# kkoutini/PaSST

Measured on AMD Instinct MI355X. Metric: clips/s (10s@32k) fwd+bwd passt_s, higher is better.
Workload: dtype bf16; 1 GPU; passt_s_swa_p16_128_ap476 train step (mel front end + mixup + fwd + BCE + bwd + adamw), 768/12/12, 474 tokens (s_patchout_t=40,f=4), random-init weights; global_batch=64, per_gpu_batch=64, parallelism=dp1, gemm_launch=persistent, 256 workgroups, input=waveform (B,1,320000) f32 resident in HBM

## Files before the change

### passt_amd/csrc/gemm.hip

```cpp
#include <algorithm>
#include <cstring>
#include <type_traits>

#include "pa_mma.h"

namespace pa {

static constexpr int NT_GROUP_M = 4;
static constexpr int BM = 128, BN = 128, KB = 128;
static constexpr int TILE_BYTES = BM * KB;
static constexpr int GEMM_LDS = 2 * 2 * TILE_BYTES;

#ifdef PA_PROBE
__device__ unsigned long long* g_probe_buf = nullptr;
static constexpr int PROBE_SLOTS = 512;
#define PA_PROBE_STAMP(cond, idx)                                                                             \
    do {                                                                                                      \
        if ((cond) && (wave & 3) == 0 && lane == 0 && (idx) < PROBE_SLOTS)                                    \
            ((unsigned long long*)(smem + G::LDS))[(wave >> 2) * PROBE_SLOTS + (idx)] = __builtin_amdgcn_s_memtime(); \
    } while (0)
#define PA_PROBE_FLAG(a, bit) (((a).reserved >> (bit)) & 1)
#define PA_PROBE_STAMP_TN(cond, idx)                                                                          \
    do {                                                                                                      \
        if ((cond) && (wave & 3) == 0 && lane == 0 && (idx) < PROBE_SLOTS)                                    \
// ... 588 lines not shown
        const int col = (c >> 1) * 32 + (c & 1) * 16 + 8 * h;
        const bool ok = col < ncols && !PA_PROBE_FLAG(a, 0);
        vo[c] = ok ? (uint32_t)q * ld2 + (uint32_t)col * 2u : V2_OOB;
        vo2[c] = ok ? (uint32_t)q * ld2b + (uint32_t)col * 2u : V2_OOB;
    }
    f32x4 b4[2][4];
#pragma unroll
    for (int j = 0; j < 2; ++j)
#pragma unroll
        for (int g = 0; g < 4; ++g) {
            b4[j][g] = f32x4{0.f, 0.f, 0.f, 0.f};
            if constexpr (EPI != PA_EPI_DGELU) {
                if (bias_row) b4[j][g] = *(const f32x4*)(bias_row + wc * 64 + j * 32 + 8 * g + 4 * h);
            }
        }
    float cs = 1.f;
    if constexpr (EPI == PA_EPI_STORE) {
        if (nb < a.colscale_n) {
            cs = a.colscale;
#pragma unroll
            for (int j = 0; j < 2; ++j)
#pragma unroll
                for (int g = 0; g < 4; ++g) b4[j][g] *= cs;
        }
    }
    constexpr int XD = V3Aux<EPI, TM>::PASSES > 0 ? V3Aux<EPI, TM>::PASSES : 1;
#pragma unroll
    for (int i = 0; i < TM; ++i) {
        __builtin_amdgcn_sched_barrier(0);
        uint32_t xg[2][4][2];
        if constexpr (EPI == PA_EPI_DGELU) {
#pragma unroll
            for (int c = 0; c < 4; ++c) {
                const u32x4 x = aux.v[(i % XD) * 4 + c];
                const int j = c >> 1, gp = c & 1;
                xg[j][2 * gp][0] = swap32_lo(x[0], x[2], xg[j][2 * gp + 1][0]);
                xg[j][2 * gp][1] = swap32_lo(x[1], x[3], xg[j][2 * gp + 1][1]);
            }
            __builtin_amdgcn_sched_barrier(0);
            if (i + XD < TM) aux.load_pass(i % XD, i + XD);
        }
#pragma unroll
        for (int j = 0; j < 2; ++j) {
            uint32_t w[4][2], w2[4][2];
#pragma unroll
            for (int g = 0; g < 4; ++g)
#pragma unroll
                for (int e2 = 0; e2 < 2; ++e2) {
                    const int r = 4 * g + 2 * e2;
                    f32x2 v = {acc[i][j][r] + b4[j][g][2 * e2], acc[i][j][r + 1] + b4[j][g][2 * e2 + 1]};
                    if constexpr (EPI == PA_EPI_STORE) v = f32x2{fmaf(acc[i][j][r], cs, b4[j][g][2 * e2]), fmaf(acc[i][j][r + 1], cs, b4[j][g][2 * e2 + 1])};
                    if constexpr (EPI == PA_EPI_DGELU) {
                        const uint32_t xw = xg[j][g][e2];
                        const f32x2 x = {__builtin_bit_cast(float, xw << 16), __builtin_bit_cast(float, xw & 0xffff0000u)};
                        v = v * (PA_PROBE_FLAG(a, 2) ? x : gelu_grad_fast2(x));
                    }
                    w[g][e2] = cvt_pk_bf16(v[0], v[1]);
                    if constexpr (EPI == PA_EPI_GELU) {
                        const f32x2 gl = PA_PROBE_FLAG(a, 2) ? v : gelu_fast2(v);
                        w2[g][e2] = cvt_pk_bf16(gl[0], gl[1]);
                    }
                }
#pragma unroll
            for (int gp = 0; gp < 2; ++gp) {
                uint32_t o0, o1;
                const uint32_t k0 = swap32_lo(w[2 * gp][0], w[2 * gp + 1][0], o0), k1 = swap32_lo(w[2 * gp][1], w[2 * gp + 1][1], o1);
                __builtin_amdgcn_raw_buffer_store_b128(u32x4{k0, k1, o0, o1}, ors, vo[2 * j + gp] + (uint32_t)(i * 32) * ld2, 0, 0);
                if constexpr (EPI == PA_EPI_GELU) {
                    const uint32_t g0 = swap32_lo(w2[2 * gp][0], w2[2 * gp + 1][0], o0), g1 = swap32_lo(w2[2 * gp][1], w2[2 * gp + 1][1], o1);
                    __builtin_amdgcn_raw_buffer_store_b128(u32x4{g0, g1, o0, o1}, ors2, vo2[2 * j + gp] + (uint32_t)(i * 32) * ld2b, 0, 0);
                }
            }
        }
    }
}

template <int TM, bool RS = false>
__device__ __forceinline__ void gemm_epilogue_v3_resid(const pa_gemm_args& a, f32x16 (&acc)[TM][2], const float* bias_row,
                                                       int m0, int n0, int wr, int wc, int lane, V3Aux<PA_EPI_RESID, TM, RS>& aux) {
    const int h = lane >> 5, q = lane & 31;
    const int mb = m0 + wr * (TM * 32), nb = n0 + wc * 64;
    if (mb >= a.M || nb >= a.N) return;
    const int ncols = a.N - nb;
    const uint32_t ldo4 = (uint32_t)a.ldo32 * 4u;
    const auto ors = tile_rsrc((const char*)a.out_f32 + ((int64_t)mb * a.ldo32 + nb) * 4, ((int64_t)(a.M - mb - 1) * a.ldo32 + ncols) * 4);
    uint32_t vo[4];
#pragma unroll
    for (int g = 0; g < 4; ++g) vo[g] = (uint32_t)q * ldo4 + (uint32_t)(8 * g + 4 * h) * 4u;
    constexpr int NH = 2 * TM, DEPTH = V3Aux<PA_EPI_RESID, TM, RS>::HALVES;
#pragma unroll
    for (int hp = 0; hp < NH; ++hp) {
        const int i = hp >> 1, j = hp & 1;
        __builtin_amdgcn_sched_barrier(0);
        f32x4 o[4];
        float f = 1.f;
        if constexpr (RS) f = __shfl(aux.rsv[i >> 1], (i & 1) * 32 + q, 64);
#pragma unroll
        for (int g = 0; g < 4; ++g) {
            const f32x4 b = bias_row ? *(const f32x4*)(bias_row + wc * 64 + j * 32 + 8 * g + 4 * h) : f32x4{0.f, 0.f, 0.f, 0.f};
            const f32x4 r = __builtin_bit_cast(f32x4, aux.v[(hp % DEPTH) * 4 + g]);
            const f32x4 ab = f32x4{acc[i][j][4 * g] + b[0], acc[i][j][4 * g + 1] + b[1], acc[i][j][4 * g + 2] + b[2], acc[i][j][4 * g + 3] + b[3]};
            if constexpr (RS) o[g] = __builtin_elementwise_fma(f32x4{f, f, f, f}, ab, r);
            else o[g] = ab + r;
        }
        __builtin_amdgcn_sched_barrier(0);
        if (hp + DEPTH < NH) aux.load_half(hp % DEPTH, hp + DEPTH, ncols);
#pragma unroll
        for (int g = 0; g < 4; ++g) {
            const uint32_t off = (j * 32 + 8 * g + 4 * h < ncols && !PA_PROBE_FLAG(a, 0)) ? vo[g] + (uint32_t)(i * 32) * ldo4 + (uint32_t)j * 128u : V2_OOB;
            __builtin_amdgcn_raw_buffer_store_b128(__builtin_bit_cast(u32x4, o[g]), ors, off, 0, 0);
        }
    }
}

template <int N> __device__ __forceinline__ void wait_vmcnt() { asm volatile("s_waitcnt vmcnt(%0)" ::"n"(N) : "memory"); }
template <int PER> __device__ __forceinline__ void wait_vm_groups(int k) {
    switch (k) {
        case 0: wait_vmcnt<0>(); break;
        case 1: wait_vmcnt<PER>(); break;
        case 2: wait_vmcnt<2 * PER>(); break;
        default: wait_vmcnt<3 * PER>(); break;
    }
}

__device__ __forceinline__ void tile_coords(int pid, int tiles_m, int tiles_n, int group_m, int& tm, int& tn) {
    const int per_group = group_m * tiles_n;
    const int g = pid / per_group;
    const int first = g * group_m;
    const int gm = min(tiles_m - first, group_m);
    const int r = pid - g * per_group;
    tm = first + r % gm;
    tn = r / gm;
}

template <int KBT> __device__ __forceinline__ int swz_rows(int row) {
    if constexpr (KBT == 128) return swz_f128(row);
    else return (row >> 2) & 3;
}

struct pa_gemm_args_rs : pa_gemm_args {
    const float* rowscale;
};
template <bool RS> using gemm_kargs = std::conditional_t<RS, pa_gemm_args_rs, pa_gemm_args>;
static constexpr int EPI_RESID_ROWSCALE = 5;
__host__ __device__ constexpr bool epi_rs(int epix) { return epix == EPI_RESID_ROWSCALE; }
__host__ __device__ constexpr int epi_base(int epix) { return epix == EPI_RESID_ROWSCALE ? (int)PA_EPI_RESID : epix; }
template <bool RS> __device__ __forceinline__ const float* rowscale_of(const gemm_kargs<RS>& a) {
    if constexpr (RS) return a.rowscale;
    else return nullptr;
}

template <typename T, int EPIX, int WM, int WN, int TM, int STAGES, int KBT = KB, int EPV = 0>
__global__ __launch_bounds__(WM * WN * 64) __attribute__((amdgpu_waves_per_eu((KBT == 64 || EPV) ? 2 : 1))) void gemm_nt_kernel(const gemm_kargs<epi_rs(EPIX)> a, const int tiles_m, const int tiles_n,
                                                               const int nwg, const int ksteps_per_split) {
    constexpr bool RS = epi_rs(EPIX);
    constexpr int EPI = epi_base(EPIX);
    static_assert(!RS || EPV == 0, "row factors: the first-generation epilogue");
    constexpr int TBM = WM * TM * 32, TBN = WN * 64;
    constexpr int A_BYTES = TBM * KBT, B_BYTES = TBN * KBT, STAGE_BYTES = A_BYTES + B_BYTES;
    constexpr int CPR = KBT / 16, NSUB = KBT / 32;
    constexpr int NW = WM * WN;
    constexpr int A_PER = (A_BYTES / 1024) / NW;
    constexpr int B_PER = (B_BYTES / 1024) / NW;
    constexpr int PER = A_PER + B_PER;
    static_assert(A_PER * NW * 1024 == A_BYTES && B_PER * NW * 1024 == B_BYTES, "tile must split evenly over the waves");
    extern __shared__ __attribute__((aligned(16))) char smem[];
    const int tid = threadIdx.x;
    const int lane = tid & 63;
    const int wave = __builtin_amdgcn_readfirstlane(tid >> 6);
    const int wr = wave / WN, wc = wave % WN;

    int tm, tn;
    tile_coords(xcd_swizzle(blockIdx.x, nwg), tiles_m, tiles_n, 1024 / TBM, tm, tn);
    const int m0 = tm * TBM, n0 = tn * TBN;
    const int ksteps_total = (int)((int64_t)a.K * sizeof(T) / KBT);
    const int ks_begin = blockIdx.y * ksteps_per_split;
    const int ks_end = min(ksteps_total, ks_begin + ksteps_per_split);
    const int nsteps = ks_end - ks_begin;

    const char* srcA[A_PER];
    const char* srcB[B_PER];
#pragma unroll
    for (int i = 0; i < A_PER; ++i) {
        const int q = (wave * A_PER + i) * 64 + lane;
        const int row = q / CPR;
        const int c = (q % CPR) ^ swz_rows<KBT>(row);
        const int gm = min(m0 + row, a.M - 1);
        srcA[i] = (const char*)a.A + ((int64_t)gm * a.lda) * sizeof(T) + c * 16 + (int64_t)ks_begin * KBT;
    }
#pragma unroll
    for (int i = 0; i < B_PER; ++i) {
        const int q = (wave * B_PER + i) * 64 + lane;
        const int row = q / CPR;
        const int c = (q % CPR) ^ swz_rows<KBT>(row);
        const int gn = min(n0 + row, a.N - 1);
        srcB[i] = (const char*)a.B + ((int64_t)gn * a.ldb) * sizeof(T) + c * 16 + (int64_t)ks_begin * KBT;
    }
    auto stage = [&](int buf, int step) {
        char* sA = smem + buf * STAGE_BYTES + wave * (A_PER * 1024);
        char* sB = smem + buf * STAGE_BYTES + A_BYTES + wave * (B_PER * 1024);
#pragma unroll
        for (int i = 0; i < A_PER; ++i)
            __builtin_amdgcn_global_load_lds(
                (const __attribute__((address_space(1))) void*)(srcA[i] + (int64_t)step * KBT),
                (__attribute__((address_space(3))) void*)(sA + i * 1024), 16, 0, 0);
#pragma unroll
        for (int i = 0; i < B_PER; ++i)
            __builtin_amdgcn_global_load_lds(
                (const __attribute__((address_space(1))) void*)(srcB[i] + (int64_t)step * KBT),
                (__attribute__((address_space(3))) void*)(sB + i * 1024), 16, 0, 0);
    };

    f32x16 acc[TM][2];
#pragma unroll
    for (int i = 0; i < TM; ++i)
#pragma unroll
        for (int j = 0; j < 2; ++j)
#pragma unroll
            for (int r = 0; r < 16; ++r) acc[i][j][r] = 0.f;

    const int rsw = swz_rows<KBT>(lane & 31);
    const int offA = (wr * (TM * 32) + (lane & 31)) * KBT;
    const int offB = (wc * 64 + (lane & 31)) * KBT;
    const int half = lane >> 5;

#pragma unroll
    for (int p = 0; p < STAGES - 1; ++p)
        if (p < nsteps) stage(p, p);
    float bias8[8];
    load_bias8<EPI>(a, n0, wc, lane, bias8);
    int buf = 0;
    for (int t = 0; t < nsteps; ++t) {
        wait_vm_groups<PER>(min(STAGES - 2, nsteps - 1 - t));
        __builtin_amdgcn_s_barrier();
        if (t + STAGES - 1 < nsteps) {
            int nb = buf + STAGES - 1;
            if (nb >= STAGES) nb -= STAGES;
            stage(nb, t + STAGES - 1);
        }
        const char* sA = smem + buf * STAGE_BYTES;
        const char* sB = sA + A_BYTES;
        typename Frag<T>::type fa[2][TM], fb[2][2];
        auto read_frags = [&](int slot, int ks) {
            const int coff = ((ks * 2 + half) ^ rsw) << 4;
#pragma unroll
            for (int i = 0; i < TM; ++i) fa[slot][i] = *(const typename Frag<T>::type*)(sA + offA + i * 32 * KBT + coff);
#pragma unroll
            for (int j = 0; j < 2; ++j) fb[slot][j] = *(const typename Frag<T>::type*)(sB + offB + j * 32 * KBT + coff);
        };
        read_frags(0, 0);
#pragma unroll
        for (int ks = 0; ks < NSUB; ++ks) {
            if (ks + 1 < NSUB) read_frags((ks + 1) & 1, ks + 1);
#pragma unroll
            for (int i = 0; i < TM; ++i)
#pragma unroll
                for (int j = 0; j < 2; ++j) mma32<T>(acc[i][j], fa[ks & 1][i], fb[ks & 1][j]);
        }
        if (++buf == STAGES) buf = 0;
    }
    if constexpr (EPV != 0) {
        constexpr bool BLK = EPV == 2;
        static_assert(sizeof(T) == 2 && EPI != PA_EPI_PARTIAL, "epilogue v2: bf16 operands, fused epilogues");
        static_assert(!BLK || EPI == PA_EPI_GELU || EPI == PA_EPI_DGELU, "blocked pre-activation: GELU / GELU' only");
        constexpr bool BLKX = BLK && (EPI == PA_EPI_GELU || EPI == PA_EPI_DGELU);
        V2Aux<EPI, TM, BLKX> aux;
        aux.issue(a, m0, n0, wr, wc, lane);
        __syncthreads();
        const float* brow = (EPI != PA_EPI_DGELU && a.bias) ? a.bias + n0 : nullptr;
        if constexpr (EPI == PA_EPI_RESID) gemm_epilogue_v2_resid<TM>(a, acc, smem + wave * 8192, brow, m0, n0, wr, wc, lane, aux);
        else gemm_epilogue_v2_bf16<EPI, TM, BLKX>(a, acc, smem + wave * 8192, brow, m0, n0, wr, wc, lane, tm * WM + wr, aux);
    } else {
        __syncthreads();
        gemm_epilogue<T, EPI, TM, RS>(a, acc, (float*)(smem + wave * SLAB_BYTES), m0, n0, blockIdx.y, wr, wc, lane, bias8, tm * WM + wr, rowscale_of<RS>(a));
    }
}

template <typename T, int EPI, int WM, int WN, int TM, int STAGES, int KBT = KB, int EPV = 0, bool RS = false>
static int launch_gemm_v(const gemm_kargs<RS>& a, hipStream_t st) {
    constexpr int TBM = WM * TM * 32, TBN = WN * 64;
    constexpr int LDS = STAGES * (TBM + TBN) * KBT;
    static_assert(LDS <= 160 * 1024, "LDS ring too large");
    static_assert(LDS >= WM * WN * 32 * 68 * 4, "epilogue slabs must fit");
    if constexpr (EPV != 0) {
        const int64_t lim = (int64_t)1 << 31;
        if ((int64_t)a.M * a.ldolp * 2 >= lim || (int64_t)a.M * a.ldolp2 * 2 >= lim || (int64_t)a.M * a.ldaux * 2 >= lim ||
            (int64_t)a.M * a.ldr * 4 >= lim || (int64_t)a.M * a.ldo32 * 4 >= lim || a.N % 64 || (EPI == PA_EPI_RESID && a.row_mod > 0))
            return EPV == 2 ? PA_EUNSUPPORTED : launch_gemm_v<T, EPI, WM, WN, TM, STAGES, KBT, 0>(a, st);
    }
    const int tiles_m = (int)cdiv(a.M, TBM), tiles_n = (int)cdiv(a.N, TBN);
    const int nwg = tiles_m * tiles_n;
    const int ksteps = (int)((int64_t)a.K * sizeof(T) / KBT);
    const int splits = EPI == PA_EPI_PARTIAL ? a.split_k : 1;
    const int per = (int)cdiv(ksteps, splits);
    static signed char lds_attr[64] = {0};
    static_assert(!RS || EPI == PA_EPI_RESID, "row factors: the residual epilogue only");
    constexpr int EPIX = RS ? EPI_RESID_ROWSCALE : EPI;
    (void)lds_attr_on_this_device((const void*)gemm_nt_kernel<T, EPIX, WM, WN, TM, STAGES, KBT, EPV>, LDS, lds_attr);
    hipLaunchKernelGGL((gemm_nt_kernel<T, EPIX, WM, WN, TM, STAGES, KBT, EPV>), dim3(nwg, splits), dim3(WM * WN * 64), LDS, st, a,
                       tiles_m, tiles_n, nwg, per);
    const int rc = check_launch();
    if (rc == PA_OK && EPI == PA_EPI_DGELU && a.colsum_out) return finish_gemm_colsum(a, tiles_m * WM, st);
    return rc;
}

template <int TM, bool A3> struct StaggerGeom {
    static constexpr int TBM = 64 * TM, TBN = 256;
    static constexpr int A_BYTES = TBM * KB, B_BYTES = TBN * KB, STAGE_BYTES = A_BYTES + B_BYTES;
    static constexpr int NA = A3 ? 3 : 2;
    static constexpr int RING = NA * A_BYTES + 2 * B_BYTES;
    __host__ __device__ static constexpr int a_off(int s) { return A3 ? s * A_BYTES : s * STAGE_BYTES; }
    __host__ __device__ static constexpr int b_off(int s) { return A3 ? 3 * A_BYTES + s * B_BYTES : s * STAGE_BYTES + A_BYTES; }
    static constexpr int SLAB = A3 ? 8192 : SLAB_BYTES;
    static constexpr int SLABS_IN_STAGE = STAGE_BYTES / SLAB_BYTES;
    static constexpr int SLABS_A = A_BYTES / 8192, SLABS_B = B_BYTES / 8192;
    static constexpr int EXTRA = A3 ? 8 - SLABS_A - SLABS_B : 8 - SLABS_IN_STAGE;
    static constexpr int BIAS_OFF = RING + EXTRA * SLAB;
    static constexpr int TAB_OFF = BIAS_OFF + 1024;
    static constexpr int MAX_ROUNDS = A3 ? 128 : 512;
    static constexpr int LDS = TAB_OFF + MAX_ROUNDS * 16;
};

template <typename T, int EPIX, int TM, bool A3 = false, bool BLK = false, bool TR = false>
__global__ __launch_bounds__(512) void gemm_nt_stagger_kernel(const gemm_kargs<epi_rs(EPIX)> a, const int tiles_m, const int tiles_n,
                                                              const int nwg, const int ksteps_per_split, const int total) {
    constexpr bool RS = epi_rs(EPIX);
    constexpr int EPI = epi_base(EPIX);
    using G = StaggerGeom<TM, A3>;
    static_assert(!RS || (sizeof(T) == 2 && EPI == PA_EPI_RESID && !BLK), "row factors: the bf16 residual epilogues (v2 / v3)");
    static_assert(!TR || (sizeof(T) == 2 && EPI != PA_EPI_PARTIAL && !BLK), "v3: bf16 operands, fused epilogues, row-major pre-activation");
    constexpr int WN = 4;
    constexpr int TBM = G::TBM, TBN = G::TBN;
    constexpr int A_PER = TM;
    constexpr int NA = G::NA, PDA = NA - 1;
    constexpr bool USE_V2 = sizeof(T) == 2 && EPI != PA_EPI_PARTIAL;
    static_assert(!A3 || (TM <= 3 && (USE_V2 || EPI == PA_EPI_PARTIAL)), "A3: LDS budget / 8 KiB slabs");
    extern __shared__ __attribute__((aligned(16))) char smem[];
    const int tid = threadIdx.x;
    const int lane = tid & 63;
    const int wave = __builtin_amdgcn_readfirstlane(tid >> 6);
    const int wr = wave / WN, wc = wave % WN;
    const int ksteps_total = (int)((int64_t)a.K * sizeof(T) / KB);
    const int nres = gridDim.x, bid = blockIdx.x;

    const int full_rounds = total / nres;
    const int my_rounds = full_rounds + (bid < total - full_rounds * nres ? 1 : 0);
    int4* tab = (int4*)(smem + G::TAB_OFF);
    for (int r = tid; r < my_rounds; r += 512) {
        const int n = min(total - r * nres, nres);
        const int item = r * nres + xcd_swizzle(bid, n);
        int tm, tn;
        const int sp = item / nwg;
        tile_coords(item - sp * nwg, tiles_m, tiles_n, NT_GROUP_M, tm, tn);
        tab[r] = make_int4(tm * TBM, tn * TBN, sp, 0);
    }
#ifdef PA_PROBE
    for (int i = tid; i < 2 * PROBE_SLOTS; i += 512) ((unsigned long long*)(smem + G::LDS))[i] = 0ull;
#endif
    __syncthreads();
    const char* baseA;
    const char* baseB;
    uint32_t voffA[A_PER], voffB[4];
    auto item_of = [&](int r, int& m0, int& n0, int& split) {
        const int4 e = tab[r];
        m0 = __builtin_amdgcn_readfirstlane(e.x);
        n0 = __builtin_amdgcn_readfirstlane(e.y);
        split = __builtin_amdgcn_readfirstlane(e.z);
        const int ks_begin = split * ksteps_per_split;
        return min(ksteps_total, ks_begin + ksteps_per_split) - ks_begin;
    };
    auto point_A = [&](int r) {
        int m0, n0, split;
        item_of(r, m0, n0, split);
        baseA = (const char*)a.A + (int64_t)m0 * a.lda * sizeof(T) + (int64_t)split * ksteps_per_split * KB;
#pragma unroll
        for (int i = 0; i < A_PER; ++i) {
            const int q = (wave * A_PER + i) * 64 + lane;
            const int row = q >> 3;
            const int c = (q & 7) ^ swz_f128(row);
            voffA[i] = (uint32_t)min(row, a.M - 1 - m0) * (uint32_t)(a.lda * (int)sizeof(T)) + c * 16;
        }
    };
    auto point_B = [&](int r) {
        int m0, n0, split;
        item_of(r, m0, n0, split);
        baseB = (const char*)a.B + (int64_t)n0 * a.ldb * sizeof(T) + (int64_t)split * ksteps_per_split * KB;
#pragma unroll
        for (int i = 0; i < 4; ++i) {
            const int q = (wave * 4 + i) * 64 + lane;
            const int row = q >> 3;
            const int c = (q & 7) ^ swz_f128(row);
            voffB[i] = (uint32_t)min(row, a.N - 1 - n0) * (uint32_t)(a.ldb * (int)sizeof(T)) + c * 16;
        }
    };
    auto dmaA = [&](int slot, int step) {
        char* sA = smem + G::a_off(slot) + wave * (A_PER * 1024);
        const char* sb = baseA + (int64_t)step * KB;
        (void)a;
#pragma unroll
        for (int i = 0; i < A_PER; ++i)
            __builtin_amdgcn_global_load_lds((const __attribute__((address_space(1))) void*)(sb + voffA[i]),
                                             (__attribute__((address_space(3))) void*)(sA + i * 1024), 16, 0, EPI == PA_EPI_RESID ? CP_DMA_A_RESID : 0);
    };
    auto dmaB = [&](int slot, int step) {
        char* sB = smem + G::b_off(slot) + wave * 4096;
        const char* sb = baseB + (int64_t)step * KB;
#pragma unroll
        for (int i = 0; i < 4; ++i)
            __builtin_amdgcn_global_load_lds((const __attribute__((address_space(1))) void*)(sb + voffB[i]),
                                             (__attribute__((address_space(3))) void*)(sB + i * 1024), 16, 0, 0);
    };

    const int rsw = swz_f128(lane);
    const int offA = (wr * (TM * 32) + (lane & 31)) * 128;
    const int offB = (wc * 64 + (lane & 31)) * 128;
    const int half = lane >> 5;

    int round = 0;
    int m0, n0, split;
    int nsteps = item_of(0, m0, n0, split);
    point_A(0);
    point_B(0);
    dmaA(0, 0);
    if constexpr (A3) dmaA(1, 1);
    dmaB(0, 0);
    asm volatile("s_waitcnt vmcnt(0)" ::: "memory");
    __builtin_amdgcn_s_barrier();
    int ia = 0, ib = 0;

    for (;;) {
        const bool have_next = round + 1 < my_rounds;
        constexpr bool HAS_BIAS = EPI != PA_EPI_PARTIAL && EPI != PA_EPI_DGELU;
        if constexpr (HAS_BIAS) {
            if (a.bias && wr == 0)
                __builtin_amdgcn_global_load_lds((const __attribute__((address_space(1))) void*)(a.bias + min(n0 + wc * 64 + lane, a.N - 1)),
                                                 (__attribute__((address_space(3))) void*)(smem + G::BIAS_OFF + wc * 256), 4, 0, 0);
        }
        f32x16 acc[TM][2];
        constexpr int AUX_EPI = USE_V2 ? EPI : PA_EPI_STORE;
        std::conditional_t<TR, V3Aux<AUX_EPI, TM, RS>, V2Aux<AUX_EPI, TM, BLK, RS>> aux;
        constexpr int AUXN = decltype(aux)::N;
        static_assert(V3Aux<AUX_EPI, TM, RS>::N == V2Aux<AUX_EPI, TM, false, RS>::N, "both epilogues leave the same number of loads in flight");
        const int cur_m0 = m0, cur_n0 = n0, cur_split = split;
        if (wr == 1) __builtin_amdgcn_s_barrier();
        PA_PROBE_STAMP(round < 24, round * 16);

        for (int t = 0; t < nsteps; ++t) {
            const char* sA = smem + G::a_off(ia);
            const char* sB = smem + G::b_off(ib);
            const bool last = t + 1 == nsteps;
            const bool fetchB = !last || have_next;
            if (last && have_next) point_B(round + 1);
            const int stepB = last ? 0 : t + 1;
            const int ta = t + PDA;
            const bool fetchA = ta < nsteps || have_next;
            if (ta == nsteps && have_next) point_A(round + 1);
            const int stepA = ta < nsteps ? ta : ta - nsteps;
            int slotA = ia + PDA;
            if (slotA >= NA) slotA -= NA;
            const int tail = (A3 && fetchA ? A_PER : 0) + (USE_V2 && AUXN > 0 && last ? AUXN : 0);
            auto wait_tile = [&]() {
                if (tail == 0) asm volatile("s_waitcnt vmcnt(0)" ::: "memory");
                else if (tail == A_PER) wait_vmcnt<A_PER>();
                else if (tail == AUXN) wait_vmcnt<(AUXN > 0 ? AUXN : 1)>();
                else wait_vmcnt<A_PER + AUXN>();
            };
            constexpr int NPH = 4;
#pragma unroll
            for (int ph = 0; ph < NPH; ++ph) {
                typename Frag<T>::type fa[TM], fb[2];
                const int coff = ((ph * 2 + half) ^ rsw) << 4;
#pragma unroll
                for (int i = 0; i < TM; ++i) fa[i] = *(const typename Frag<T>::type*)(sA + offA + i * 32 * 128 + coff);
#pragma unroll
                for (int j = 0; j < 2; ++j) fb[j] = *(const typename Frag<T>::type*)(sB + offB + j * 32 * 128 + coff);
                if constexpr (A3) {
                    if (ph == 0 && fetchB) dmaB(ib ^ 1, stepB);
                    if (ph == 1 && fetchA) dmaA(slotA, stepA);
                } else {
                    if (ph == 0 && fetchA) dmaA(slotA, stepA);
                    if (ph == 1 && fetchB) dmaB(ib ^ 1, stepB);
                }
                if constexpr (USE_V2 && AUXN > 0) {
                    if (last && ph == NPH / 2) aux.issue(a, cur_m0, cur_n0, wr, wc, lane, rowscale_of<RS>(a));
                }
                if (ph == NPH - 1 && wr == 1) wait_tile();
                asm volatile("s_waitcnt lgkmcnt(0)" ::: "memory");
                __builtin_amdgcn_sched_barrier(0);
                __builtin_amdgcn_s_barrier();
                __builtin_amdgcn_s_setprio(1);
                if (ph == 0 && t == 0) {
#pragma unroll
                    for (int i = 0; i < TM; ++i)
#pragma unroll
                        for (int j = 0; j < 2; ++j) mma32_first<T>(acc[i][j], TR ? fb[j] : fa[i], TR ? fa[i] : fb[j]);
                } else {
#pragma unroll
                    for (int i = 0; i < TM; ++i)
#pragma unroll
                        for (int j = 0; j < 2; ++j) mma32<T>(acc[i][j], TR ? fb[j] : fa[i], TR ? fa[i] : fb[j]);
                }
                __builtin_amdgcn_s_setprio(0);
                if (ph == NPH - 1 && wr == 0) wait_tile();
                __builtin_amdgcn_sched_barrier(0);
                __builtin_amdgcn_s_barrier();
            }
            if (++ia == NA) ia = 0;
            ib ^= 1;
            PA_PROBE_STAMP(round < 24 && t < 13, round * 16 + 1 + t);
        }
        if (wr == 0) __builtin_amdgcn_s_barrier();
        const int freeA = ia == 0 ? NA - 1 : ia - 1, freeB = ib ^ 1;
        char* slab_c;
        if constexpr (A3) {
            slab_c = wave < G::SLABS_A ? smem + G::a_off(freeA) + wave * 8192
                     : wave < G::SLABS_A + G::SLABS_B ? smem + G::b_off(freeB) + (wave - G::SLABS_A) * 8192
                                                      : smem + G::RING + (wave - G::SLABS_A - G::SLABS_B) * 8192;
        } else {
            slab_c = wave < G::SLABS_IN_STAGE ? smem + G::a_off(freeA) + wave * SLAB_BYTES
                                              : smem + G::RING + (wave - G::SLABS_IN_STAGE) * SLAB_BYTES;
        }
        float* slab = (float*)slab_c;
        if (PA_PROBE_FLAG(a, 1)) {
#pragma unroll
            for (int i = 0; i < TM; ++i)
#pragma unroll
                for (int j = 0; j < 2; ++j)
#pragma unroll
                    for (int r = 0; r < 16; ++r) asm volatile("" ::"v"(acc[i][j][r]));
        } else if constexpr (USE_V2) {
            const float* brow = HAS_BIAS && a.bias ? (const float*)(smem + G::BIAS_OFF) : nullptr;
            if constexpr (TR) {
                (void)slab;
                if constexpr (EPI == PA_EPI_RESID) gemm_epilogue_v3_resid<TM, RS>(a, acc, brow, cur_m0, cur_n0, wr, wc, lane, aux);
                else gemm_epilogue_v3_bf16<EPI, TM>(a, acc, brow, cur_m0, cur_n0, wr, wc, lane, aux);
            } else if constexpr (EPI == PA_EPI_RESID) gemm_epilogue_v2_resid<TM, RS>(a, acc, (char*)slab, brow, cur_m0, cur_n0, wr, wc, lane, aux);
            else gemm_epilogue_v2_bf16<EPI, TM, BLK>(a, acc, (char*)slab, brow, cur_m0, cur_n0, wr, wc, lane, (cur_m0 / TBM) * 2 + wr, aux);
        } else if constexpr (EPI == PA_EPI_RESID || EPI == PA_EPI_PARTIAL) {
            (void)slab;
            gemm_epilogue_f32_direct<EPI, TM>(a, acc, HAS_BIAS && a.bias ? (const float*)(smem + G::BIAS_OFF) : nullptr, cur_m0,
                                              cur_n0, cur_split, wr, wc, lane);
        } else {
            float bias8[8];
#pragma unroll
            for (int e = 0; e < 8; ++e) bias8[e] = 0.f;
            if constexpr (HAS_BIAS) {
                if (a.bias) {
                    const float* brow = (const float*)(smem + G::BIAS_OFF) + wc * 64 + (lane & 7) * 8;
                    const f32x4 lo = *(const f32x4*)brow, hi = *(const f32x4*)(brow + 4);
#pragma unroll
                    for (int e = 0; e < 4; ++e) { bias8[e] = lo[e]; bias8[4 + e] = hi[e]; }
                }
            }
            gemm_epilogue<T, EPI, TM>(a, acc, slab, cur_m0, cur_n0, cur_split, wr, wc, lane, bias8, (cur_m0 / TBM) * 2 + wr);
        }
        PA_PROBE_STAMP(round < 24, round * 16 + 15);
#ifdef PA_PROBE
        if (!have_next && g_probe_buf && blockIdx.x < 8) {
            __syncthreads();
            for (int i = tid; i < 2 * PROBE_SLOTS; i += 512)
                g_probe_buf[blockIdx.x * 2 * PROBE_SLOTS + i] = ((const unsigned long long*)(smem + G::LDS))[i];
        }
#endif
        if (!have_next) break;
        ++round;
        nsteps = item_of(round, m0, n0, split);
        point_A(round);
        point_B(round);
        asm volatile("s_waitcnt lgkmcnt(0)" ::: "memory");
        __builtin_amdgcn_s_barrier();
    }
}

static bool epilogue_v3_enabled() {
    static const bool on = [] { const char* e = getenv("PA_EPILOGUE_V3"); return e && atoi(e) != 0; }();
    return on;
}

template <typename T, int EPI, int TM, bool A3 = false, bool BLK = false, bool TR = false, bool RS = false>
static int launch_gemm_stagger(const gemm_kargs<RS>& a, hipStream_t st) {
    using G = StaggerGeom<TM, A3>;
    if constexpr (!TR && !BLK && sizeof(T) == 2 && EPI != PA_EPI_PARTIAL && !(EPI == PA_EPI_RESID && TM == 4)) {
        if ((epilogue_v3_enabled() || (a.reserved & PA_GEMM_EPILOGUE_V3)) && !(EPI == PA_EPI_DGELU && a.colsum_out) &&
            !(EPI == PA_EPI_RESID && a.row_mod > 0))
            return launch_gemm_stagger<T, EPI, TM, A3, false, true, RS>(a, st);
    }
    static_assert(G::LDS <= 160 * 1024, "LDS budget");
    const int tiles_m = (int)cdiv(a.M, 64 * TM), tiles_n = (int)cdiv(a.N, 256);
    const int nwg = tiles_m * tiles_n;
    const int ksteps = (int)((int64_t)a.K * sizeof(T) / KB);
    const int splits = EPI == PA_EPI_PARTIAL ? a.split_k : 1;
    const int per = (int)cdiv(ksteps, splits);
    const int total = nwg * splits;
    const int64_t lim = (int64_t)1 << 31;
    const bool big = (int64_t)a.M * a.ldolp * 2 >= lim || (int64_t)a.M * a.ldolp2 * 2 >= lim || (int64_t)a.M * a.ldaux * 2 >= lim ||
                     (int64_t)a.M * a.ldr * 4 >= lim || (int64_t)a.M * a.ldo32 * 4 >= lim;
    if (ksteps < 1 || (int64_t)(splits - 1) * per >= ksteps ||
        (sizeof(T) == 2 && EPI != PA_EPI_PARTIAL && (big || (EPI == PA_EPI_RESID && a.row_mod > 0))))
        return BLK ? PA_EUNSUPPORTED : launch_gemm_v<T, EPI, 2, 2, 2, 2, KB, 0, RS>(a, st);
    if constexpr (A3) {
        if (ksteps - (splits - 1) * per < 2 || per < 2 || cdiv(total, 256) > G::MAX_ROUNDS) return launch_gemm_stagger<T, EPI, TM, false, BLK, TR, RS>(a, st);
    } else {
        if (cdiv(total, 256) > G::MAX_ROUNDS) return BLK ? PA_EUNSUPPORTED : launch_gemm_v<T, EPI, 2, 2, 2, 2, KB, 0, RS>(a, st);
    }
#ifdef PA_PROBE
    constexpr int LDS_BYTES = G::LDS + 2 * PROBE_SLOTS * 8;
#else
    constexpr int LDS_BYTES = G::LDS;
#endif
    static_assert(LDS_BYTES <= 160 * 1024, "LDS budget (probe build)");
    static signed char lds_attr[64] = {0};
    static_assert(!RS || EPI == PA_EPI_RESID, "row factors: the residual epilogue only");
    constexpr int EPIX = RS ? EPI_RESID_ROWSCALE : EPI;
    (void)lds_attr_on_this_device((const void*)gemm_nt_stagger_kernel<T, EPIX, TM, A3, BLK, TR>, LDS_BYTES, lds_attr);
    static const bool persist_env = [] { const char* e = getenv("PA_NT_PERSISTENT"); return !e || atoi(e) != 0; }();
    const bool persistent = persist_env && !(a.reserved & PA_GEMM_NO_PERSIST);
    hipLaunchKernelGGL((gemm_nt_stagger_kernel<T, EPIX, TM, A3, BLK, TR>), dim3(persistent ? std::min(total, 256) : total), dim3(512), LDS_BYTES, st, a,
                       tiles_m, tiles_n, nwg, per, total);
    const int rc = check_launch();
    if (rc == PA_OK && EPI == PA_EPI_DGELU && a.colsum_out) return finish_gemm_colsum(a, tiles_m * 2, st);
    return rc;
}

static int pick_nt_variant(int M, int N, int K) {
    struct Cand { int id, bm, bn, slots; float rate_short, rate_long; };
    static const Cand r06[] = {
        {1, 128, 128, 512, 700.f, 870.f},
        {8, 128, 256, 256, 800.f, 950.f},
        {7, 192, 256, 256, 950.f, 1075.f},
        {6, 256, 256, 256, 930.f, 900.f},
    };
    static const Cand r01[] = {
        {1, 128, 128, 512, 750.f, 930.f},
        {8, 128, 256, 256, 650.f, 1000.f},
        {7, 192, 256, 256, 780.f, 1250.f},
        {6, 256, 256, 256, 800.f, 1150.f},
    };
    static const bool isolated_table = [] { const char* e = getenv("PA_NT_RATES"); return e && !strcmp(e, "r06"); }();
    const Cand (&cands)[4] = isolated_table ? r06 : r01;
    int best = 1;
    double best_cost = 1e30;
    for (const Cand& c : cands) {
        const int64_t tiles = cdiv(M, c.bm) * cdiv(N, c.bn);
        const double rounds = (double)cdiv(tiles, c.slots);
        const double rate = (K <= 1024 ? c.rate_short : c.rate_long) / c.slots;
        const double cost = rounds * (double)c.bm * c.bn / rate;
        if (cost < best_cost) { best_cost = cost; best = c.id; }
    }
    return best;
}

template <typename T, int EPI>
static int launch_gemm(const pa_gemm_args& a, hipStream_t st) {
    if constexpr (sizeof(T) == 4) return launch_gemm_v<T, EPI, 2, 2, 2, 2>(a, st);
    else {
        int v = a.tune ? a.tune : pick_nt_variant(a.M, a.N, a.K);
        static const bool a3 = [] { const char* e = getenv("PA_NT_A3"); return !e || atoi(e) != 0; }();
        if (!a.tune && a3 && EPI != PA_EPI_PARTIAL && (v == 7 || v == 8)) v += 10;
        if constexpr (EPI == PA_EPI_GELU || EPI == PA_EPI_DGELU) {
            if (a.reserved & PA_GEMM_BLOCKED_PRE) {
                if (a.N % 64 || blocked_pre_rows(a.M) * a.N * 2 >= ((int64_t)1 << 31)) return PA_EUNSUPPORTED;
                static const bool mlp_2wg = [] { const char* e = getenv("PA_NT_MLP_2WG"); return e && atoi(e) != 0; }();
                if (!a.tune && mlp_2wg && a.M >= 16384 && a.N >= 1024 && a.K <= (EPI == PA_EPI_DGELU ? 1024 : 768)) v = 3;
                switch (v) {
                    case 6: return launch_gemm_stagger<T, EPI, 4, false, true>(a, st);
                    case 7: return launch_gemm_stagger<T, EPI, 3, false, true>(a, st);
                    case 8: return launch_gemm_stagger<T, EPI, 2, false, true>(a, st);
                    case 17: return launch_gemm_stagger<T, EPI, 3, true, true>(a, st);
                    case 18: return launch_gemm_stagger<T, EPI, 2, true, true>(a, st);
                    case 3: return launch_gemm_v<T, EPI, 2, 2, 3, 2, KB, 2>(a, st);
                    case 9: return launch_gemm_v<T, EPI, 1, 4, 4, 3, 64, 2>(a, st);
                }
                return PA_EUNSUPPORTED;
            }
        }
        switch (v) {
            case 1: return launch_gemm_v<T, EPI, 2, 2, 2, 2>(a, st);
            case 2: return launch_gemm_v<T, EPI, 2, 4, 4, 2>(a, st);
            case 3: return launch_gemm_v<T, EPI, 2, 2, 3, 2>(a, st);
            case 9: return launch_gemm_v<T, EPI, 1, 4, 4, 3, 64>(a, st);
            case 13: if constexpr (EPI != PA_EPI_PARTIAL) return launch_gemm_v<T, EPI, 2, 2, 3, 2, KB, 1>(a, st); else return PA_EINVAL;
            case 19: if constexpr (EPI != PA_EPI_PARTIAL) return launch_gemm_v<T, EPI, 1, 4, 4, 3, 64, 1>(a, st); else return PA_EINVAL;
            case 6: return launch_gemm_stagger<T, EPI, 4>(a, st);
            case 7: return launch_gemm_stagger<T, EPI, 3>(a, st);
            case 8: return launch_gemm_stagger<T, EPI, 2>(a, st);
            case 17: return launch_gemm_stagger<T, EPI, 3, true>(a, st);
            case 18: return launch_gemm_stagger<T, EPI, 2, true>(a, st);
        }
        return PA_EINVAL;
    }
}

template <typename T>
static int launch_gemm_rs(const pa_gemm_args_rs& a, hipStream_t st) {
    if constexpr (sizeof(T) == 4) return launch_gemm_v<T, PA_EPI_RESID, 2, 2, 2, 2, KB, 0, true>(a, st);
    else {
        int v = a.tune;
        if (v != 1 && v != 6 && v != 7 && v != 8 && v != 17 && v != 18) {
            v = pick_nt_variant(a.M, a.N, a.K);
            static const bool a3 = [] { const char* e = getenv("PA_NT_A3"); return !e || atoi(e) != 0; }();
            if (a3 && (v == 7 || v == 8)) v += 10;
        }
        switch (v) {
            case 1: return launch_gemm_v<T, PA_EPI_RESID, 2, 2, 2, 2, KB, 0, true>(a, st);
            case 6: return launch_gemm_stagger<T, PA_EPI_RESID, 4, false, false, false, true>(a, st);
            case 7: return launch_gemm_stagger<T, PA_EPI_RESID, 3, false, false, false, true>(a, st);
            case 8: return launch_gemm_stagger<T, PA_EPI_RESID, 2, false, false, false, true>(a, st);
            case 17: return launch_gemm_stagger<T, PA_EPI_RESID, 3, true, false, false, true>(a, st);
            case 18: return launch_gemm_stagger<T, PA_EPI_RESID, 2, true, false, false, true>(a, st);
        }
        return PA_EINVAL;
    }
}

template <typename T> struct TNGeom {
    static constexpr int COLS = 128;
    static constexpr int ROWB = COLS * (int)sizeof(T);
    static constexpr int MROWS = TILE_BYTES / ROWB;
    static constexpr int RPI = 1024 / ROWB;
    static constexpr int LPR = ROWB / 16;
    static constexpr int EPC = 16 / (int)sizeof(T);
    static constexpr int FSTEP = Frag<T>::K;
};

template <typename T> __device__ __forceinline__ int tn_swz(int row, int c) {
    if constexpr (sizeof(T) == 2) return row * 256 + ((c ^ ((row & 3) << 2)) << 4);
    else return row * 512 + (c << 4);
}

template <typename T>
__device__ __forceinline__ typename Frag<T>::type tn_frag(const char* tile, int ms, int cbase, int lane);
template <>
__device__ __forceinline__ bf16x8 tn_frag<bf16>(const char* tile, int ms, int cbase, int lane) {
    const int p = lane & 15, g = (lane >> 4) & 1, h = lane >> 5;
    const int r1 = ms * 16 + h * 8 + (p >> 2);
    const int col = cbase + g * 16 + (p & 3) * 4;
    const int within = (col & 7) * 2;
    const bf16x4 lo = lds_tr16(tile + tn_swz<bf16>(r1, col >> 3) + within);
    const bf16x4 hi = lds_tr16(tile + tn_swz<bf16>(r1 + 4, col >> 3) + within);
    bf16x8 f;
    f[0] = lo[0]; f[1] = lo[1]; f[2] = lo[2]; f[3] = lo[3];
    f[4] = hi[0]; f[5] = hi[1]; f[6] = hi[2]; f[7] = hi[3];
    return f;
}
template <>
__device__ __forceinline__ f32x4 tn_frag<float>(const char* tile, int ms, int cbase, int lane) {
    const int col = cbase + (lane & 31), h = lane >> 5;
    f32x4 f;
#pragma unroll
    for (int e = 0; e < 4; ++e) f[e] = *(const float*)(tile + (ms * 8 + h * 4 + e) * 512 + col * 4);
    return f;
}

template <typename T>
__global__ __launch_bounds__(256) void gemm_tn_kernel(const pa_gemm_args a, const int tiles_n, const int nwg,
                                                      const int steps_per_split) {
    using G = TNGeom<T>;
    extern __shared__ __attribute__((aligned(16))) char smem[];
    const int tid = threadIdx.x;
    const int lane = tid & 63;
    const int wave = __builtin_amdgcn_readfirstlane(tid >> 6);
    const int wr = wave >> 1, wc = wave & 1;
    const int bid = xcd_swizzle(blockIdx.x, nwg);
    const int m0 = (bid / tiles_n) * BM, n0 = (bid % tiles_n) * BN;
    const int Mtok = a.K;
    const int steps_total = (Mtok + G::MROWS - 1) / G::MROWS;
    const int st_begin = blockIdx.y * steps_per_split;
    const int st_end = min(steps_total, st_begin + steps_per_split);
    const int nsteps = st_end - st_begin;

    const char* srcA[4];
    const char* srcB[4];
    int rowin[4];
#pragma unroll
    for (int i = 0; i < 4; ++i) {
        const int q = wave * 4 + i;
        const int row = q * G::RPI + lane / G::LPR;
        const int pc = lane % G::LPR;
        const int c = sizeof(T) == 2 ? (pc ^ ((row & 3) << 2)) : pc;
        rowin[i] = row;
        const int ca = min(m0 + c * G::EPC, a.M - G::EPC), cb = min(n0 + c * G::EPC, a.N - G::EPC);
        srcA[i] = (const char*)a.A + (int64_t)ca * sizeof(T);
        srcB[i] = (const char*)a.B + (int64_t)cb * sizeof(T);
    }
    auto stage = [&](int buf, int step) {
        char* sA = smem + buf * (2 * TILE_BYTES) + wave * 4096;
        char* sB = sA + TILE_BYTES;
#pragma unroll
        for (int i = 0; i < 4; ++i) {
            const int64_t tok = min((int64_t)(st_begin + step) * G::MROWS + rowin[i], (int64_t)Mtok - 1);
            __builtin_amdgcn_global_load_lds(
                (const __attribute__((address_space(1))) void*)(srcA[i] + tok * a.lda * sizeof(T)),
                (__attribute__((address_space(3))) void*)(sA + i * 1024), 16, 0, 0);
            __builtin_amdgcn_global_load_lds(
                (const __attribute__((address_space(1))) void*)(srcB[i] + tok * a.ldb * sizeof(T)),
                (__attribute__((address_space(3))) void*)(sB + i * 1024), 16, 0, 0);
        }
    };
    auto zero_tail = [&](int buf, int step) {
        const int valid = Mtok - (st_begin + step) * G::MROWS;
        if (valid >= G::MROWS) return;
        char* sA = smem + buf * (2 * TILE_BYTES);
        char* sB = sA + TILE_BYTES;
#pragma unroll
        for (int i = 0; i < 4; ++i) {
            if (rowin[i] >= valid) {
                const int off = (wave * 4 + i) * 1024 + lane * 16;
                *(uint4*)(sA + off) = make_uint4(0, 0, 0, 0);
                *(uint4*)(sB + off) = make_uint4(0, 0, 0, 0);
            }
        }
    };

    f32x16 acc[2][2];
#pragma unroll
    for (int i = 0; i < 2; ++i)
#pragma unroll
        for (int j = 0; j < 2; ++j)
#pragma unroll
            for (int r = 0; r < 16; ++r) acc[i][j][r] = 0.f;

    if (nsteps > 0) stage(0, 0);
    for (int t = 0; t < nsteps; ++t) {
        asm volatile("s_waitcnt vmcnt(0)" ::: "memory");
        zero_tail(t & 1, t);
        __syncthreads();
        if (t + 1 < nsteps) stage((t + 1) & 1, t + 1);
        const char* sA = smem + (t & 1) * (2 * TILE_BYTES);
        const char* sB = sA + TILE_BYTES;
#pragma unroll
        for (int ms = 0; ms < G::MROWS / G::FSTEP; ++ms) {
            typename Frag<T>::type fa[2], fb[2];
#pragma unroll
            for (int i = 0; i < 2; ++i) {
                fa[i] = tn_frag<T>(sA, ms, wr * 64 + i * 32, lane);
                fb[i] = tn_frag<T>(sB, ms, wc * 64 + i * 32, lane);
            }
#pragma unroll
            for (int i = 0; i < 2; ++i)
#pragma unroll
                for (int j = 0; j < 2; ++j) mma32<T>(acc[i][j], fa[i], fb[j]);
        }
    }
    __syncthreads();
    const float nobias[8] = {0.f, 0.f, 0.f, 0.f, 0.f, 0.f, 0.f, 0.f};
    gemm_epilogue<T, PA_EPI_PARTIAL, 2>(a, acc, (float*)(smem + wave * SLAB_BYTES), m0, n0, blockIdx.y, wr, wc, lane, nobias);
}

__device__ __forceinline__ int tn2_swz(int row, int c) { return row * 512 + ((c ^ ((row & 3) << 2)) << 4); }

__device__ __forceinline__ bf16x8 tn2_frag(const char* tile, int ms, int cbase, int lane) {
    const int p = lane & 15, g = (lane >> 4) & 1, h = lane >> 5;
    const int r1 = ms * 16 + h * 8 + (p >> 2);
    const int col = cbase + g * 16 + (p & 3) * 4;
    const int within = (col & 7) * 2;
    const bf16x4 lo = lds_tr16(tile + tn2_swz(r1, col >> 3) + within);
    const bf16x4 hi = lds_tr16(tile + tn2_swz(r1 + 4, col >> 3) + within);
// ... 1016 lines not shown
```

### passt_amd/csrc/pa_mma.h

```cpp
#pragma once
#include "pa_common.h"

namespace pa {

template <typename T> struct Frag;
template <> struct Frag<bf16> { typedef bf16x8 type; static constexpr int K = 16; };
template <> struct Frag<float> { typedef f32x4 type; static constexpr int K = 8; };

template <typename T>
__device__ __forceinline__ void mma32(f32x16& acc, const typename Frag<T>::type& a,
                                      const typename Frag<T>::type& b);
template <>
__device__ __forceinline__ void mma32<bf16>(f32x16& acc, const bf16x8& a, const bf16x8& b) {
    acc = __builtin_amdgcn_mfma_f32_32x32x16_bf16(a, b, acc, 0, 0, 0);
}
template <>
__device__ __forceinline__ void mma32<float>(f32x16& acc, const f32x4& a, const f32x4& b) {
#pragma unroll
    for (int e = 0; e < 4; ++e) acc = __builtin_amdgcn_mfma_f32_32x32x2f32(a[e], b[e], acc, 0, 0, 0);
}

template <typename T>
__device__ __forceinline__ void mma32_first(f32x16& acc, const typename Frag<T>::type& a, const typename Frag<T>::type& b);
template <>
__device__ __forceinline__ void mma32_first<bf16>(f32x16& acc, const bf16x8& a, const bf16x8& b) {
    const f32x16 z = {0.f, 0.f, 0.f, 0.f, 0.f, 0.f, 0.f, 0.f, 0.f, 0.f, 0.f, 0.f, 0.f, 0.f, 0.f, 0.f};
    acc = __builtin_amdgcn_mfma_f32_32x32x16_bf16(a, b, z, 0, 0, 0);
}
template <>
__device__ __forceinline__ void mma32_first<float>(f32x16& acc, const f32x4& a, const f32x4& b) {
    const f32x16 z = {0.f, 0.f, 0.f, 0.f, 0.f, 0.f, 0.f, 0.f, 0.f, 0.f, 0.f, 0.f, 0.f, 0.f, 0.f, 0.f};
    acc = __builtin_amdgcn_mfma_f32_32x32x2f32(a[0], b[0], z, 0, 0, 0);
#pragma unroll
    for (int e = 1; e < 4; ++e) acc = __builtin_amdgcn_mfma_f32_32x32x2f32(a[e], b[e], acc, 0, 0, 0);
}

template <typename T>
__device__ __forceinline__ void mma32_c(f32x16& acc, const typename Frag<T>::type& a, const typename Frag<T>::type& b, const f32x16& c);
template <>
__device__ __forceinline__ void mma32_c<bf16>(f32x16& acc, const bf16x8& a, const bf16x8& b, const f32x16& c) {
    acc = __builtin_amdgcn_mfma_f32_32x32x16_bf16(a, b, c, 0, 0, 0);
}
template <>
__device__ __forceinline__ void mma32_c<float>(f32x16& acc, const f32x4& a, const f32x4& b, const f32x16& c) {
    acc = __builtin_amdgcn_mfma_f32_32x32x2f32(a[0], b[0], c, 0, 0, 0);
#pragma unroll
    for (int e = 1; e < 4; ++e) acc = __builtin_amdgcn_mfma_f32_32x32x2f32(a[e], b[e], acc, 0, 0, 0);
}

__device__ __forceinline__ int acc_row(int r, int lane) { return (r & 3) + 8 * (r >> 2) + 4 * (lane >> 5); }

__device__ __forceinline__ int swz_f128(int row) {
    const int y = (row >> 1) & 7;
    return ((y & 1) << 2) | (y & 2) | (y >> 2);
}
__device__ __forceinline__ int swz128(int row, int c) { return row * 128 + ((c ^ swz_f128(row)) << 4); }
__device__ __forceinline__ int swz256(int row, int c) { return row * 256 + ((c ^ (row & 15)) << 4); }

template <int ROWBYTES> __device__ __forceinline__ int swz(int row, int c) {
    if constexpr (ROWBYTES == 128) return swz128(row, c);
    else return swz256(row, c);
}

template <typename T> __device__ __forceinline__ typename Frag<T>::type acc_frag(const f32x16& p, int s);
template <> __device__ __forceinline__ bf16x8 acc_frag<bf16>(const f32x16& p, int s) {
    bf16x8 f;
#pragma unroll
    for (int j = 0; j < 8; ++j) f[j] = (bf16)p[8 * s + j];
    return f;
}
template <> __device__ __forceinline__ f32x4 acc_frag<float>(const f32x16& p, int s) {
    f32x4 f;
#pragma unroll
    for (int e = 0; e < 4; ++e) f[e] = p[4 * s + e];
    return f;
}
template <typename T> struct AccSteps;
template <> struct AccSteps<bf16> { static constexpr int N = 2; };
template <> struct AccSteps<float> { static constexpr int N = 4; };

__device__ __forceinline__ bf16x4 lds_tr16(const char* lds_ptr) {
    typedef __attribute__((__vector_size__(4 * sizeof(__bf16)))) __bf16 v4;
    v4 r = __builtin_amdgcn_ds_read_tr16_b64_v4bf16(
        (__attribute__((address_space(3))) v4*)(lds_ptr));
    bf16x4 o;
    o[0] = r[0]; o[1] = r[1]; o[2] = r[2]; o[3] = r[3];
    return o;
}

template <int OFF>
__device__ __forceinline__ bf16x4 lds_tr16_asm(uint32_t lds_addr) {
    typedef uint32_t u32x2 __attribute__((ext_vector_type(2)));
    u32x2 r;
    asm volatile("ds_read_b64_tr_b16 %0, %1 offset:%2" : "=v"(r) : "v"(lds_addr), "n"(OFF));
    return __builtin_bit_cast(bf16x4, r);
}
__device__ __forceinline__ bf16x4 lds_tr16_asm_imm(uint32_t lds_addr, int off) {
    typedef uint32_t u32x2 __attribute__((ext_vector_type(2)));
    u32x2 r;
    asm volatile("ds_read_b64_tr_b16 %0, %1 offset:%2" : "=v"(r) : "v"(lds_addr), "i"(off));
    return __builtin_bit_cast(bf16x4, r);
}

}
```

Measured before the change: 2952 clips/s.

## Use 16x16x32 bf16 MFMA in the staggered NT GEMM with lane remap

```diff
diff --git a/passt_amd/csrc/gemm.hip b/passt_amd/csrc/gemm.hip
--- a/passt_amd/csrc/gemm.hip
+++ b/passt_amd/csrc/gemm.hip
@@ -914,6 +914,17 @@
     const int rc = check_launch();
     if (rc == PA_OK && EPI == PA_EPI_DGELU && a.colsum_out) return finish_gemm_colsum(a, tiles_m * WM, st);
     return rc;
+}
+
+#ifdef PA_NT_MFMA32
+template <typename T> constexpr bool NT_MFMA16 = false;
+#else
+template <typename T> constexpr bool NT_MFMA16 = sizeof(T) == 2;
+#endif
+static constexpr int NT16_PHASES = 4;
+template <typename T> __device__ __forceinline__ int nt_swz(int row) {
+    if constexpr (NT_MFMA16<T>) return swz_nt128(row);
+    else return swz_f128(row);
 }
 
 template <int TM, bool A3> struct StaggerGeom {
@@ -989,7 +1000,7 @@
         for (int i = 0; i < A_PER; ++i) {
             const int q = (wave * A_PER + i) * 64 + lane;
             const int row = q >> 3;
-            const int c = (q & 7) ^ swz_f128(row);
+            const int c = (q & 7) ^ nt_swz<T>(row);
             voffA[i] = (uint32_t)min(row, a.M - 1 - m0) * (uint32_t)(a.lda * (int)sizeof(T)) + c * 16;
         }
     };
@@ -1001,7 +1012,7 @@
         for (int i = 0; i < 4; ++i) {
             const int q = (wave * 4 + i) * 64 + lane;
             const int row = q >> 3;
-            const int c = (q & 7) ^ swz_f128(row);
+            const int c = (q & 7) ^ nt_swz<T>(row);
             voffB[i] = (uint32_t)min(row, a.N - 1 - n0) * (uint32_t)(a.ldb * (int)sizeof(T)) + c * 16;
         }
     };
@@ -1027,6 +1038,14 @@
     const int offA = (wr * (TM * 32) + (lane & 31)) * 128;
     const int offB = (wc * 64 + (lane & 31)) * 128;
     const int half = lane >> 5;
+    constexpr bool M16 = NT_MFMA16<T>;
+    const int rA16 = TR ? (lane & 15) : perm16(lane & 15), rB16 = TR ? perm16(lane & 15) : (lane & 15);
+    int offA16[2], offB16[2];
+#pragma unroll
+    for (int s = 0; s < 2; ++s) {
+        offA16[s] = (wr * (TM * 32) + rA16) * 128 + (((4 * s + (lane >> 4)) ^ swz_nt128(rA16)) << 4);
+        offB16[s] = (wc * 64 + rB16) * 128 + (((4 * s + (lane >> 4)) ^ swz_nt128(rB16)) << 4);
+    }
 
     int round = 0;
     int m0, n0, split;
@@ -1049,10 +1068,13 @@
                                                  (__attribute__((address_space(3))) void*)(smem + G::BIAS_OFF + wc * 256), 4, 0, 0);
         }
         f32x16 acc[TM][2];
+        int lane_e = lane;
+        if constexpr (M16) asm volatile("" : "+v"(lane_e));
         constexpr int AUX_EPI = USE_V2 ? EPI : PA_EPI_STORE;
         std::conditional_t<TR, V3Aux<AUX_EPI, TM, RS>, V2Aux<AUX_EPI, TM, BLK, RS>> aux;
         constexpr int AUXN = decltype(aux)::N;
         static_assert(V3Aux<AUX_EPI, TM, RS>::N == V2Aux<AUX_EPI, TM, false, RS>::N, "both epilogues leave the same number of loads in flight");
+        constexpr bool AUX_LATE = NT_MFMA16<T> && USE_V2 && AUXN > 0 && (TM == 4 || (TR && RS));
         const int cur_m0 = m0, cur_n0 = n0, cur_split = split;
         if (wr == 1) __builtin_amdgcn_s_barrier();
         PA_PROBE_STAMP(round < 24, round * 16);
@@ -1070,38 +1092,72 @@
             const int stepA = ta < nsteps ? ta : ta - nsteps;
             int slotA = ia + PDA;
             if (slotA >= NA) slotA -= NA;
-            const int tail = (A3 && fetchA ? A_PER : 0) + (USE_V2 && AUXN > 0 && last ? AUXN : 0);
+            const int tail = (A3 && fetchA ? A_PER : 0) + (USE_V2 && AUXN > 0 && !AUX_LATE && last ? AUXN : 0);
             auto wait_tile = [&]() {
                 if (tail == 0) asm volatile("s_waitcnt vmcnt(0)" ::: "memory");
                 else if (tail == A_PER) wait_vmcnt<A_PER>();
                 else if (tail == AUXN) wait_vmcnt<(AUXN > 0 ? AUXN : 1)>();
                 else wait_vmcnt<A_PER + AUXN>();
             };
-            constexpr int NPH = 4;
+            constexpr int NPH = M16 ? NT16_PHASES : 4;
+            static_assert(NPH == 2 || NPH == 4, "phase pairs per K-tile");
+            constexpr int PH_DMA1 = NPH == 2 ? 0 : 1;
+            constexpr int PPS = NPH / 2;
+            constexpr int NG = 2 * TM / PPS;
+            bf16x8 fa16[NG], fb16[4];
 #pragma unroll
             for (int ph = 0; ph < NPH; ++ph) {
                 typename Frag<T>::type fa[TM], fb[2];
-                const int coff = ((ph * 2 + half) ^ rsw) << 4;
-#pragma unroll
-                for (int i = 0; i < TM; ++i) fa[i] = *(const typename Frag<T>::type*)(sA + offA + i * 32 * 128 + coff);
-#pragma unroll
-                for (int j = 0; j < 2; ++j) fb[j] = *(const typename Frag<T>::type*)(sB + offB + j * 32 * 128 + coff);
+                if constexpr (M16) {
+                    const int s = ph / PPS, g0 = (ph % PPS) * NG;
+#pragma unroll
+                    for (int x = 0; x < NG; ++x) fa16[x] = *(const bf16x8*)(sA + offA16[s] + (g0 + x) * 16 * 128);
+                    if (ph % PPS == 0) {
+#pragma unroll
+                        for (int b = 0; b < 4; ++b) fb16[b] = *(const bf16x8*)(sB + offB16[s] + b * 16 * 128);
+                    }
+                } else {
+                    const int coff = ((ph * 2 + half) ^ rsw) << 4;
+#pragma unroll
+                    for (int i = 0; i < TM; ++i) fa[i] = *(const typename Frag<T>::type*)(sA + offA + i * 32 * 128 + coff);
+#pragma unroll
+                    for (int j = 0; j < 2; ++j) fb[j] = *(const typename Frag<T>::type*)(sB + offB + j * 32 * 128 + coff);
+                }
                 if constexpr (A3) {
                     if (ph == 0 && fetchB) dmaB(ib ^ 1, stepB);
-                    if (ph == 1 && fetchA) dmaA(slotA, stepA);
+                    if (ph == PH_DMA1 && fetchA) dmaA(slotA, stepA);
                 } else {
                     if (ph == 0 && fetchA) dmaA(slotA, stepA);
-                    if (ph == 1 && fetchB) dmaB(ib ^ 1, stepB);
+                    if (ph == PH_DMA1 && fetchB) dmaB(ib ^ 1, stepB);
                 }
                 if constexpr (USE_V2 && AUXN > 0) {
-                    if (last && ph == NPH / 2) aux.issue(a, cur_m0, cur_n0, wr, wc, lane, rowscale_of<RS>(a));
+                    if (!AUX_LATE && last && ph == NPH / 2) aux.issue(a, cur_m0, cur_n0, wr, wc, lane_e, rowscale_of<RS>(a));
                 }
                 if (ph == NPH - 1 && wr == 1) wait_tile();
                 asm volatile("s_waitcnt lgkmcnt(0)" ::: "memory");
                 __builtin_amdgcn_sched_barrier(0);
                 __builtin_amdgcn_s_barrier();
                 __builtin_amdgcn_s_setprio(1);
-                if (ph == 0 && t == 0) {
+                if constexpr (M16) {
+                    const int g0 = (ph % PPS) * NG;
+                    if (ph < PPS && t == 0) {
+#pragma unroll
+                        for (int x = 0; x < NG; ++x)
+#pragma unroll
+                            for (int b = 0; b < 4; ++b) {
+                                const int ga = g0 + x, pa = ga & 1, qb = b & 1;
+                                mma16_slice<true>(acc[ga >> 1][b >> 1], TR ? 2 * qb + pa : 2 * pa + qb, TR ? fb16[b] : fa16[x], TR ? fa16[x] : fb16[b]);
+                            }
+                    } else {
+#pragma unroll
+                        for (int x = 0; x < NG; ++x)
+#pragma unroll
+                            for (int b = 0; b < 4; ++b) {
+                                const int ga = g0 + x, pa = ga & 1, qb = b & 1;
+                                mma16_slice<false>(acc[ga >> 1][b >> 1], TR ? 2 * qb + pa : 2 * pa + qb, TR ? fb16[b] : fa16[x], TR ? fa16[x] : fb16[b]);
+                            }
+                    }
+                } else if (ph == 0 && t == 0) {
 #pragma unroll
                     for (int i = 0; i < TM; ++i)
 #pragma unroll
@@ -1121,7 +1177,14 @@
             ib ^= 1;
             PA_PROBE_STAMP(round < 24 && t < 13, round * 16 + 1 + t);
         }
+        if constexpr (AUX_LATE) aux.issue(a, cur_m0, cur_n0, wr, wc, lane_e, rowscale_of<RS>(a));
         if (wr == 0) __builtin_amdgcn_s_barrier();
+        if constexpr (M16) {
+#pragma unroll
+            for (int i = 0; i < TM; ++i)
+#pragma unroll
+                for (int j = 0; j < 2; ++j) acc32_from_16(acc[i][j]);
+        }
         const int freeA = ia == 0 ? NA - 1 : ia - 1, freeB = ib ^ 1;
         char* slab_c;
         if constexpr (A3) {
@@ -1144,27 +1207,27 @@
             const float* brow = HAS_BIAS && a.bias ? (const float*)(smem + G::BIAS_OFF) : nullptr;
             if constexpr (TR) {
                 (void)slab;
-                if constexpr (EPI == PA_EPI_RESID) gemm_epilogue_v3_resid<TM, RS>(a, acc, brow, cur_m0, cur_n0, wr, wc, lane, aux);
-                else gemm_epilogue_v3_bf16<EPI, TM>(a, acc, brow, cur_m0, cur_n0, wr, wc, lane, aux);
-            } else if constexpr (EPI == PA_EPI_RESID) gemm_epilogue_v2_resid<TM, RS>(a, acc, (char*)slab, brow, cur_m0, cur_n0, wr, wc, lane, aux);
-            else gemm_epilogue_v2_bf16<EPI, TM, BLK>(a, acc, (char*)slab, brow, cur_m0, cur_n0, wr, wc, lane, (cur_m0 / TBM) * 2 + wr, aux);
+                if constexpr (EPI == PA_EPI_RESID) gemm_epilogue_v3_resid<TM, RS>(a, acc, brow, cur_m0, cur_n0, wr, wc, lane_e, aux);
+                else gemm_epilogue_v3_bf16<EPI, TM>(a, acc, brow, cur_m0, cur_n0, wr, wc, lane_e, aux);
+            } else if constexpr (EPI == PA_EPI_RESID) gemm_epilogue_v2_resid<TM, RS>(a, acc, (char*)slab, brow, cur_m0, cur_n0, wr, wc, lane_e, aux);
+            else gemm_epilogue_v2_bf16<EPI, TM, BLK>(a, acc, (char*)slab, brow, cur_m0, cur_n0, wr, wc, lane_e, (cur_m0 / TBM) * 2 + wr, aux);
         } else if constexpr (EPI == PA_EPI_RESID || EPI == PA_EPI_PARTIAL) {
             (void)slab;
             gemm_epilogue_f32_direct<EPI, TM>(a, acc, HAS_BIAS && a.bias ? (const float*)(smem + G::BIAS_OFF) : nullptr, cur_m0,
-                                              cur_n0, cur_split, wr, wc, lane);
+                                              cur_n0, cur_split, wr, wc, lane_e);
         } else {
             float bias8[8];
 #pragma unroll
             for (int e = 0; e < 8; ++e) bias8[e] = 0.f;
             if constexpr (HAS_BIAS) {
                 if (a.bias) {
-                    const float* brow = (const float*)(smem + G::BIAS_OFF) + wc * 64 + (lane & 7) * 8;
+                    const float* brow = (const float*)(smem + G::BIAS_OFF) + wc * 64 + (lane_e & 7) * 8;
                     const f32x4 lo = *(const f32x4*)brow, hi = *(const f32x4*)(brow + 4);
 #pragma unroll
                     for (int e = 0; e < 4; ++e) { bias8[e] = lo[e]; bias8[4 + e] = hi[e]; }
                 }
             }
-            gemm_epilogue<T, EPI, TM>(a, acc, slab, cur_m0, cur_n0, cur_split, wr, wc, lane, bias8, (cur_m0 / TBM) * 2 + wr);
+            gemm_epilogue<T, EPI, TM>(a, acc, slab, cur_m0, cur_n0, cur_split, wr, wc, lane_e, bias8, (cur_m0 / TBM) * 2 + wr);
         }
         PA_PROBE_STAMP(round < 24, round * 16 + 15);
 #ifdef PA_PROBE
diff --git a/passt_amd/csrc/pa_mma.h b/passt_amd/csrc/pa_mma.h
--- a/passt_amd/csrc/pa_mma.h
+++ b/passt_amd/csrc/pa_mma.h
@@ -49,6 +49,29 @@
 }
 
 __device__ __forceinline__ int acc_row(int r, int lane) { return (r & 3) + 8 * (r >> 2) + 4 * (lane >> 5); }
+
+__device__ __forceinline__ int perm16(int x) { return (x & 3) | ((x & 4) << 1) | ((x & 8) >> 1); }
+
+template <bool FIRST>
+__device__ __forceinline__ void mma16_slice(f32x16& acc, int k, const bf16x8& a, const bf16x8& b) {
+    f32x4 c = {0.f, 0.f, 0.f, 0.f};
+    if constexpr (!FIRST) c = f32x4{acc[4 * k], acc[4 * k + 1], acc[4 * k + 2], acc[4 * k + 3]};
+    c = __builtin_amdgcn_mfma_f32_16x16x32_bf16(a, b, c, 0, 0, 0);
+#pragma unroll
+    for (int e = 0; e < 4; ++e) acc[4 * k + e] = c[e];
+}
+__device__ __forceinline__ void acc32_from_16(f32x16& acc) {
+#pragma unroll
+    for (int p = 0; p < 2; ++p)
+#pragma unroll
+        for (int r = 0; r < 4; ++r) {
+            const float x = acc[8 * p + r], y = acc[8 * p + 4 + r];
+            const auto s = __builtin_amdgcn_permlane16_swap(__builtin_bit_cast(unsigned, x), __builtin_bit_cast(unsigned, y), false, false);
+            acc[8 * p + r] = __builtin_bit_cast(float, (unsigned)s[0]);
+            acc[8 * p + 4 + r] = __builtin_bit_cast(float, (unsigned)s[1]);
+        }
+}
+__device__ __forceinline__ int swz_nt128(int row) { return (row >> 1) & 7; }
 
 __device__ __forceinline__ int swz_f128(int row) {
     const int y = (row >> 1) & 7;
```

After: 3050 clips/s (median of 6 runs). 1.03x the previous value.
